# YuxuanZhao/NewsRecommend

Hardware: NVIDIA B200
Metric: queries/s, top-50 IP over 364k x 250 items (flat exact search) (higher is better)
Workload: dtype f32 (fp16 tcgen05 filter with a proven error margin + exact fp32 rescoring)

## Files before the change

newsrecommend_b200/csrc/api.cu:

```cuda
#include <atomic>
#include <cstdarg>
#include <cstdlib>
#include <cstring>
#include <random>
#include <vector>

#include <cuda_fp16.h>

#include "common.cuh"
#include "internal.h"

namespace nrb {

static thread_local char g_err[512] = "";
static std::atomic<long long> g_launches{0};

void set_error(const char* fmt, ...) {
    va_list ap;
    va_start(ap, fmt);
    vsnprintf(g_err, sizeof(g_err), fmt, ap);
    va_end(ap);
}
void count_launch(int n) { g_launches += n; }

// ... 30 lines not shown
    size_t off = 0;
    explicit Carver(void* p) : base((char*)p) {}
    template <typename T>
    T* take(size_t count) {
        T* r = (T*)(base ? base + off : nullptr);
        off += align_up(count * sizeof(T), 256);
        return r;
    }
};

struct FlatPlan {
    int nqt;
    int npairs;
    int full_pairs;
    int tail_pairs;
    int tsplit;
    int chunk_rows;
    int n_units;
    int wgs;
    int S;
    int grid;
    int single;
    int pw;
};

static FlatPlan plan_flat(int64_t nq, int64_t nb, int k, int path) {
    FlatPlan p;
    p.pw = (path == NRB_PATH_TC1 || path == NRB_PATH_TC16) ? tc1_pw(k, nb > 4096) : k;
    const bool simt = path == NRB_PATH_SIMT;
    p.wgs = simt ? 1 : 2;
    p.nqt = (int)((nq + UNIT_ROWS - 1) / UNIT_ROWS);
    if (p.nqt < 1) p.nqt = 1;
    p.npairs = (p.nqt + 1) / 2;
    const int C = simt ? sm_count() : sm_count() / 2;
    const int tile = 256;
    int nbt = (int)((nb + tile - 1) / tile);
    if (nbt < 1) nbt = 1;
    p.full_pairs = (p.npairs / C) * C;
    p.tail_pairs = p.npairs - p.full_pairs;
    int best = 1;
    if (p.tail_pairs > 0) {
        int max_split = nbt < 64 ? nbt : 64;
        static const double ov_tiles = getenv("NRB_FLAT_OV_TILES") ? atof(getenv("NRB_FLAT_OV_TILES")) : 200.0;
        const double ov = ov_tiles / nbt;
        double best_cost = 1e30;
        for (int s = 1; s <= max_split; s++) {
            const double waves = (double)(((int64_t)p.tail_pairs * s + C - 1) / C);
            const double cost = waves * (1.0 / s + ov);
            if (cost < best_cost * 0.97) {
// ... 7 lines not shown
        const int C1 = sm_count();
        static const double ov_tiles1 = getenv("NRB_FLAT_OV_TILES") ? atof(getenv("NRB_FLAT_OV_TILES")) : 200.0;
        const double ov = ov_tiles1 / nbt;
        const int max_split = nbt < 64 ? nbt : 64;
        const double pair_cost = (double)(((int64_t)p.tail_pairs * best + C - 1) / C) * (1.0 / best + ov);
        int best1 = 1;
        double best_cost1 = 1e30;
        for (int s = 1; s <= max_split; s++) {
            const double waves = (double)(((int64_t)p.nqt * s + C1 - 1) / C1);
            const double cost = waves * (1.0 / s + ov);
            if (cost < best_cost1 * 0.97) {
                best_cost1 = cost;
                best1 = s;
            }
        }
        if (best_cost1 < 0.9 * pair_cost || getenv("NRB_FORCE_SINGLE_CTA")) {
            p.single = 1;
            best = best1;
        }
    }
    const int tiles_per = (nbt + best - 1) / best;
    p.chunk_rows = tiles_per * tile;
    p.tsplit = (nbt + tiles_per - 1) / tiles_per;
    p.n_units = p.single ? p.nqt * p.tsplit : 2 * (p.full_pairs + p.tail_pairs * p.tsplit);
    p.S = p.tsplit * p.wgs;
    if (p.single)
        p.grid = p.n_units < sm_count() ? p.n_units : sm_count();
    else
        p.grid = simt ? simt_grid(p.n_units) : tc_grid(p.n_units);
    return p;
}

struct FlatWs {
    Unit* units;
    int* n_units;
    int* src;
    float* part_key;
    int* part_idx;
    int* part_cnt;
    int *flags, *flag_list, *flag_count;
    unsigned* gthr;
    void* scratch;
    size_t scratch_bytes;
    size_t total;
};

static FlatWs carve_flat(void* ws, const FlatPlan& p, int64_t nq, int k, int path) {
    Carver c(ws);
    FlatWs w;
    const bool filt = path == NRB_PATH_TC1 || path == NRB_PATH_TC16;
    const int pw = p.pw;
    w.units = c.take<Unit>(p.n_units);
    w.n_units = c.take<int>(1);
// ... 361 lines not shown
    if (path == NRB_PATH_AUTO)
        path = tc16_eligible(q, b, k) ? NRB_PATH_TC16 : tc1_eligible(q, b, k) ? NRB_PATH_TC1 : NRB_PATH_TC;
    if (path == NRB_PATH_TC1 && !tc1_eligible(q, b, k)) {
        set_error("search_flat: NRB_PATH_TC1 needs raw/hi/norms planes on both sides, max_norm on the item "
                  "side, kp <= 256 and k <= %d", TC1_MAX_PW - TC1_MIN_EXTRA);
        return NRB_ERR_INVALID;
    }
    if (path == NRB_PATH_TC16 && !tc16_eligible(q, b, k)) {
        set_error("search_flat: NRB_PATH_TC16 needs raw/h16/norms planes and h16 scales on both sides, max_norm on "
                  "the item side, kp <= 256 and k <= %d", TC1_MAX_PW - TC1_MIN_EXTRA);
        return NRB_ERR_INVALID;
    }
    const bool filt = path == NRB_PATH_TC1 || path == NRB_PATH_TC16;
    if (!filt) path = resolve_path(path);
    const FlatPlan p = plan_flat(q->n, b->n, k, path);
    const FlatWs w = carve_flat(workspace, p, q->n, k, path);
    if (!workspace || workspace_bytes < w.total) {
        set_error("search_flat: workspace %zu < %zu bytes", workspace_bytes, w.total);
        return NRB_ERR_WORKSPACE;
    }
    int rc;
    if (p.single)
        rc = launch_fill_flat_units_single(w.units, w.n_units, w.src, q->n, b->n, p.nqt, p.tsplit, p.chunk_rows, p.wgs, st);
    else
        rc = launch_fill_flat_units(w.units, w.n_units, w.src, q->n, b->n, p.nqt, p.full_pairs, p.tail_pairs, p.tsplit,
                                    p.chunk_rows, p.wgs, st);
    if (rc) return rc;
    const bool seeded = seed_kth && filt && w.gthr;
    if (seeded) {
        int64_t blocks = (q->n + 255) / 256;
        if (blocks > 148 * 8) blocks = 148 * 8;
        seed_bounds_kernel<<<(unsigned)blocks, 256, 0, st>>>(seed_kth, q->n, metric == NRB_METRIC_L2 ? 1 : 0, w.gthr);
        NRB_LAUNCH_CHECK();
    } else if (w.gthr) {
        NRB_CUDA_CHECK(cudaMemsetAsync(w.gthr, 0, (size_t)q->n * sizeof(unsigned), st));
    }
    if (!filt) {
        {
            ProfScope prof(st);
            if (path == NRB_PATH_SIMT)
                rc = launch_topk_simt_dev(q, b, w.units, w.n_units, p.grid, metric, k, w.part_key, w.part_idx, w.scratch, w.scratch_bytes, st);
            else
                rc = launch_topk_tc_dev(q, b, w.units, w.n_units, p.grid, metric, k, w.part_key, w.part_idx, w.scratch,
                                        w.scratch_bytes, w.gthr, nullptr, 1, st);
        }
        if (rc) return rc;
        return launch_select(w.part_key, w.part_idx, w.src, p.S, q->n, k, metric, nullptr, id_base, D, I, st);
    }
    const int pw = p.pw;
    const float eps_xmax = TC1_EPS * b->max_norm;
    NRB_CUDA_CHECK(cudaMemsetAsync(w.flags, 0, (size_t)q->n * sizeof(int), st));
    {
        ProfScope prof(st);
        rc = launch_topk_tc1_dev(q, b, w.units, w.n_units, p.grid, metric, k, pw, 2.f * eps_xmax, w.part_key,
                                 w.part_idx, w.part_cnt, w.flags, w.scratch, w.scratch_bytes, w.gthr, nullptr, 1,
                                 path == NRB_PATH_TC16, p.single, (!p.single && b->n <= 256) ? 1 : 0, st,
                                 seeded ? 1 : 0);
    }
    if (rc) return rc;
    if ((rc = launch_gather_refine(w.part_key, w.part_idx, w.part_cnt, w.src, p.S, q->n, k, pw, metric, q, b, eps_xmax,
                                   id_base, nullptr, w.flags, D, I, st))) return rc;
    if ((rc = launch_compact_flags(w.flags, q->n, w.flag_list, w.flag_count, st))) return rc;
    if (k == 1 && b->n <= K1_FALLBACK_MAX_ROWS) {
        return launch_exact_k1_fallback(q, b, metric, id_base, w.flag_list, w.flag_count, D, I, st);
    }
    int nflag = 0;
    NRB_CUDA_CHECK(cudaMemcpyAsync(&nflag, w.flag_count, sizeof(int), cudaMemcpyDeviceToHost, st));
    NRB_CUDA_CHECK(cudaStreamSynchronize(st));
    if (nflag == 0) return NRB_OK;
    NRB_REQUIRE(b->hi && b->lo && ((q->hi && q->lo) || q->raw),
                "search_flat: %d queries need the 3xTF32 fallback but the item hi/lo planes are missing", nflag);
    g_fallback_queries += nflag;
    const size_t plane = (size_t)nflag * q->kp * sizeof(float);
    const size_t wsb2 = nrb_search_flat_workspace(nflag, b->n, k, q->kp);
    char* tmp = nullptr;
    const size_t tmp_bytes = 3 * align_up(plane, 256) + align_up((size_t)nflag * 4, 256) +
                             align_up((size_t)nflag * k * 4, 256) + align_up((size_t)nflag * k * 8, 256) + wsb2;
    keep_pool_memory();
    NRB_CUDA_CHECK(cudaMallocAsync((void**)&tmp, tmp_bytes, st));
    Carver c(tmp);
// ... 48 lines not shown
                                      size_t workspace_bytes, int32_t path, const float* seed_kth, void* stream) {
    NRB_REQUIRE(q && b && D && I, "search_flat_seeded: null argument");
    NRB_REQUIRE(metric == NRB_METRIC_INNER_PRODUCT || metric == NRB_METRIC_L2, "search_flat_seeded: bad metric %d", metric);
    NRB_REQUIRE(k >= 1 && k <= NRB_MAX_K, "search_flat_seeded: k=%d out of range [1,%d]", k, NRB_MAX_K);
    NRB_REQUIRE(q->d == b->d && q->kp == b->kp, "search_flat_seeded: dimension mismatch");
    NRB_REQUIRE(q->n >= 0 && b->n >= 0 && b->n < (1LL << 31) - 4096 && q->n < (1LL << 31), "search_flat_seeded: sizes out of range");
    NRB_REQUIRE(path >= NRB_PATH_AUTO && path <= NRB_PATH_TC16, "search_flat_seeded: bad path %d", path);
    if (q->n == 0) return NRB_OK;
    int rc = require_device();
    if (rc) return rc;
    return search_flat_impl(q, b, metric, k, id_base, D, I, workspace, workspace_bytes, path, (cudaStream_t)stream, seed_kth);
}

extern "C" int64_t nrb_fallback_query_count(void) { return (int64_t)g_fallback_queries.load(); }

extern "C" int nrb_plan_flat_describe(int64_t nq, int64_t nb, int32_t k, int32_t path, int32_t* out10) {
    NRB_REQUIRE(out10 && nq >= 1 && nb >= 0 && k >= 1 && k <= NRB_MAX_K, "plan_flat_describe: bad arguments");
    NRB_REQUIRE(path == NRB_PATH_SIMT || path == NRB_PATH_TC || path == NRB_PATH_TC1 || path == NRB_PATH_TC16,
                "plan_flat_describe: path must be a concrete path, not %d", path);
    const FlatPlan p = plan_flat(nq, nb, k, path);
    const int v[10] = {p.nqt, p.npairs, p.full_pairs, p.tail_pairs, p.tsplit, p.chunk_rows, p.n_units, p.S, p.grid, p.single};
    for (int i = 0; i < 10; i++) out10[i] = v[i];
    return NRB_OK;
}

extern "C" size_t nrb_ivf_search_workspace(int64_t nq, int32_t nprobe, int32_t k, int32_t kp,
                                           int32_t nlist, int32_t max_list_len) {
    if (nq <= 0 || nprobe <= 0 || k <= 0) return 256;
    size_t best = 0;
    for (int path : {NRB_PATH_TC, NRB_PATH_SIMT, NRB_PATH_TC16}) {
        if (path == NRB_PATH_TC16 && !tc1_k_ok(k)) continue;
        const IvfPlan p = plan_ivf(nq, nprobe, nlist, max_list_len, path);
        const size_t t = carve_ivf(nullptr, p, nlist, k, kp, path, nq).total;
        best = t > best ? t : best;
    }
    return best + 256;
}

namespace nrb {

static inline int ivf_mode_of(int nph, int i) {
    static const int force = getenv("NRB_IVF_MODE") ? atoi(getenv("NRB_IVF_MODE")) : -1;
    if (force >= 0) return force;
    return (nph > 1 && i == 1) ? 2 : 1;
}

// ... 307 lines not shown
```

newsrecommend_b200/csrc/internal.h:

```cpp
#pragma once
#include <cstdlib>
#include <cuda_runtime.h>
#include <stdint.h>

#include "../../include/nrb200.h"

namespace nrb {

struct Unit {
    int a_row0;
    int a_rows;
    int b_row0;
    int b_rows;
};

constexpr int UNIT_ROWS = 128;

int tc_available();
size_t tc_scratch_bytes(int grid);
int tc_grid(int n_units_upper);
void tc_set_variant(int v);
int launch_topk_tc_dev(const nrb_matrix* a, const nrb_matrix* b, const Unit* units,
                       const int* n_units_dev, int grid, int metric, int k, float* part_key,
                       int* part_idx, void* scratch, size_t scratch_bytes, unsigned* gthr,
                       const int* row_map, int row_div, cudaStream_t st);

constexpr int TC1_EXTRA = 32;
constexpr int TC1_EXTRA_FLAT = 96;
constexpr int TC1_MIN_EXTRA = 16;
constexpr int TC1_MAX_PW = 128;
static inline int tc1_extra() {
    static const int v = getenv("NRB_TC1_EXTRA") ? atoi(getenv("NRB_TC1_EXTRA")) : TC1_EXTRA;
    return v < TC1_MIN_EXTRA ? TC1_MIN_EXTRA : v;
}
static inline int tc1_pw(int k, bool flat = false) {
    const int extra = (flat && !getenv("NRB_TC1_EXTRA")) ? TC1_EXTRA_FLAT : tc1_extra();
    return k + extra <= TC1_MAX_PW ? k + extra : TC1_MAX_PW;
}
static inline int tc1_k_ok(int k) { return k + TC1_MIN_EXTRA <= TC1_MAX_PW; }
constexpr float TC1_EPS = 1.1f / 1024.f;
int tc1_eligible(const nrb_matrix* a, const nrb_matrix* b, int k);
int tc16_eligible(const nrb_matrix* a, const nrb_matrix* b, int k);
int launch_topk_tc1_dev(const nrb_matrix* a, const nrb_matrix* b, const Unit* units,
                        const int* n_units_dev, int grid, int metric, int k, int pw, float margin_scale,
                        float* part_key, int* part_idx, int* part_cnt, int* row_flags, void* scratch,
                        size_t scratch_bytes, unsigned* gthr, const int* row_map, int row_div, int f16,
                        int single, int ivf_mode, cudaStream_t st, int seeded = 0);

size_t simt_scratch_bytes(int grid);
int simt_grid(int n_units_upper);
int launch_topk_simt_dev(const nrb_matrix* a, const nrb_matrix* b, const Unit* units,
                         const int* n_units_dev, int grid, int metric, int k, float* part_key,
                         int* part_idx, void* scratch, size_t scratch_bytes, cudaStream_t st);

int launch_select(const float* part_key, const int* part_idx, const int* src, int S, int64_t nq,
                  int k, int metric, const int64_t* id_map, int64_t id_base, float* D, int64_t* I,
                  cudaStream_t st);
int launch_gather_refine(const float* part_key, const int* part_idx, const int* part_cnt, const int* src, int S,
                         int64_t nq, int k, int pw, int metric, const nrb_matrix* q, const nrb_matrix* b, float eps_xmax,
                         int64_t id_base, const int64_t* id_map, int* flags, float* D, int64_t* I, cudaStream_t st);
int launch_compact_flags(const int* flags, int64_t n, int* list, int* count, cudaStream_t st);
int launch_scatter_results(const float* Df, const int64_t* If, const int* list, int n, int k, float* D,
                           int64_t* I, cudaStream_t st);
int launch_fill_flat_units(Unit* units, int* n_units_out, int* src, int64_t nq, int64_t nb, int nqt,
                           int full_pairs, int tail_pairs, int tsplit, int chunk_rows, int wgs, cudaStream_t st);
int launch_fill_flat_units_single(Unit* units, int* n_units_out, int* src, int64_t nq, int64_t nb, int nqt,
                                  int tsplit, int chunk_rows, int wgs, cudaStream_t st);
size_t counting_sort_ws(int64_t n, int nb);
int launch_counting_sort_i64(const int64_t* key, int64_t n, int nb, int* offsets, int* order,
                             int* pos_of, void* ws, size_t ws_bytes, cudaStream_t st);
int launch_pack_rows(const float* x, int64_t n, int d, int64_t ldx, int kp, float* raw, float* hi, float* lo,
                     float* norms, cudaStream_t st);
int launch_gather_rows(const float* src, int width, const int32_t* idx, int div, int64_t n,
                       float* dst, cudaStream_t st);
int launch_gather_scalar(const float* src, const int32_t* idx, int div, int64_t n, float* dst,
                         cudaStream_t st);

size_t kmeans_update_ws(int64_t n, int k, int kp);
int launch_kmeans_update(const float* x_raw, int64_t n, int d, int kp, const int64_t* assign, int k, float* centroids,
                         float* hassign, void* workspace, const float* cent_in, int metric, double* obj_out,
                         cudaStream_t st, double* sums_out = nullptr);
int launch_km_split(int d, int k, int64_t n, float* hassign, float* centroids, double* stats, cudaStream_t st);

constexpr int K1_FALLBACK_MAX_ROWS = 65536;
int launch_exact_k1_fallback(const nrb_matrix* q, const nrb_matrix* b, int metric, int64_t id_base, const int* list,
                             const int* count, float* D, int64_t* I, cudaStream_t st);

int sm_count();
// ... 3 lines not shown
```

newsrecommend_b200/csrc/kernels_misc.cu:

```cuda
#include <cfloat>

#include <cuda_fp16.h>

#include "common.cuh"
#include "internal.h"

namespace nrb {

__global__ void pack_rows_kernel(const float* __restrict__ x, int64_t n, int d, int64_t ldx,
                                 int kp, float* __restrict__ raw, float* __restrict__ hi,
                                 float* __restrict__ lo, float* __restrict__ norms) {
    const int lane = threadIdx.x & 31;
    const int64_t warp0 = (int64_t)blockIdx.x * (blockDim.x >> 5) + (threadIdx.x >> 5);
    const int64_t nwarps = (int64_t)gridDim.x * (blockDim.x >> 5);
    for (int64_t row = warp0; row < n; row += nwarps) {
        const float* xr = x + row * ldx;
        float acc = 0.f;
        for (int c = lane; c < kp; c += 32) {
            float v = (c < d) ? xr[c] : 0.f;
            acc = fmaf(v, v, acc);
            const int64_t o = row * kp + c;
            if (raw) raw[o] = v;
            if (hi || lo) {
                uint32_t hb, lb;
// ... 881 lines not shown
            u.b_row0 = c * chunk_rows;
            const int64_t br = nb - (int64_t)c * chunk_rows;
            u.b_rows = (int)(br < chunk_rows ? (br > 0 ? br : 0) : chunk_rows);
        }
        units[tid] = u;
    }
    const int S = tsplit * wgs;
    const int64_t total = nq * S;
    for (int64_t e = tid; e < total; e += (int64_t)gridDim.x * blockDim.x) {
        const int64_t q = e / S;
        const int sl = (int)(e - q * S);
        const int c = sl / wgs, g = sl - c * wgs;
        const int t = (int)(q / UNIT_ROWS), pair = t >> 1, r = t & 1;
        int64_t u = -1;
        if (pair < full_pairs) {
            if (c == 0) u = 2 * (int64_t)pair + r;
        } else {
            u = 2 * ((int64_t)full_pairs + (int64_t)c * tail_pairs + (pair - full_pairs)) + r;
        }
        src[e] = u < 0 ? -1 : (int)((u * wgs + g) * UNIT_ROWS + q % UNIT_ROWS);
    }
}

__global__ void fill_flat_units_single_kernel(Unit* __restrict__ units, int* __restrict__ n_units_out,
                                              int* __restrict__ src, int64_t nq, int64_t nb, int nqt, int tsplit,
                                              int chunk_rows, int wgs) {
    const int64_t tid = (int64_t)blockIdx.x * blockDim.x + threadIdx.x;
    const int64_t nunits = (int64_t)nqt * tsplit;
    if (tid == 0) *n_units_out = (int)nunits;
    if (tid < nunits) {
        const int c = (int)(tid / nqt), t = (int)(tid - (int64_t)c * nqt);
        Unit u;
        const int64_t ar = nq - (int64_t)t * UNIT_ROWS;
        u.a_rows = (int)(ar < UNIT_ROWS ? ar : UNIT_ROWS);
        u.a_row0 = t * UNIT_ROWS;
        u.b_row0 = c * chunk_rows;
        const int64_t br = nb - (int64_t)c * chunk_rows;
        u.b_rows = (int)(br < chunk_rows ? (br > 0 ? br : 0) : chunk_rows);
        units[tid] = u;
    }
    const int S = tsplit * wgs;
    const int64_t total = nq * S;
    for (int64_t e = tid; e < total; e += (int64_t)gridDim.x * blockDim.x) {
        const int64_t q = e / S;
        const int sl = (int)(e - q * S);
        const int c = sl / wgs, g = sl - c * wgs;
// ... 50 lines not shown
    return NRB_OK;
}

int launch_scatter_results(const float* Df, const int64_t* If, const int* list, int n, int k, float* D,
                           int64_t* I, cudaStream_t st) {
    if (n == 0) return NRB_OK;
    int64_t blocks = ((int64_t)n * k + 255) / 256;
    if (blocks > 4096) blocks = 4096;
    scatter_results_kernel<<<(unsigned)blocks, 256, 0, st>>>(Df, If, list, n, k, D, I);
    NRB_LAUNCH_CHECK();
    return NRB_OK;
}

int launch_fill_flat_units(Unit* units, int* n_units_out, int* src, int64_t nq, int64_t nb, int nqt,
                           int full_pairs, int tail_pairs, int tsplit, int chunk_rows, int wgs, cudaStream_t st) {
    const int64_t total = nq * tsplit * wgs;
    const int64_t nunits = 2 * ((int64_t)full_pairs + (int64_t)tail_pairs * tsplit);
    int64_t blocks = (total + 255) / 256;
    if (blocks > 4096) blocks = 4096;
    if (blocks < (nunits + 255) / 256) blocks = (nunits + 255) / 256;
    if (blocks < 1) blocks = 1;
    fill_flat_units_kernel<<<(unsigned)blocks, 256, 0, st>>>(units, n_units_out, src, nq, nb, nqt, full_pairs,
                                                             tail_pairs, tsplit, chunk_rows, wgs);
    NRB_LAUNCH_CHECK();
    return NRB_OK;
}

int launch_fill_flat_units_single(Unit* units, int* n_units_out, int* src, int64_t nq, int64_t nb, int nqt,
                                  int tsplit, int chunk_rows, int wgs, cudaStream_t st) {
    const int64_t total = nq * tsplit * wgs;
    const int64_t nunits = (int64_t)nqt * tsplit;
    int64_t blocks = (total + 255) / 256;
    if (blocks > 4096) blocks = 4096;
    if (blocks < (nunits + 255) / 256) blocks = (nunits + 255) / 256;
    if (blocks < 1) blocks = 1;
    fill_flat_units_single_kernel<<<(unsigned)blocks, 256, 0, st>>>(units, n_units_out, src, nq, nb, nqt, tsplit,
                                                                    chunk_rows, wgs);
    NRB_LAUNCH_CHECK();
    return NRB_OK;
}

size_t counting_sort_ws(int64_t n, int nb);
int launch_counting_sort_i64(const int64_t* key, int64_t n, int nb, int* offsets, int* order,
                             int* pos_of, void* ws, size_t ws_bytes, cudaStream_t st) {
    const int nchunks = (int)((n + CS_CHUNK - 1) / CS_CHUNK);
    const size_t need = counting_sort_ws(n, nb);
// ... 364 lines not shown
```

newsrecommend_b200/csrc/topk_tc.cu:

```cuda
#include <cuda.h>

#include <cstdlib>

#include "common.cuh"
#include "internal.h"
#include "ptx.cuh"

namespace nrb {

namespace {

constexpr int BM = 128;
constexpr int BN = 256;
constexpr int KC = 32;
constexpr int A_BYTES = BM * KC * 4;
constexpr int BH_BYTES = (BN / 2) * KC * 4;
constexpr int B_BYTES = BN * KC * 4;
constexpr int NUM_THREADS = 384;
constexpr int EPI_WARP0 = 4;
constexpr int EPI_WGS = 2;
constexpr int HALF_N = BN / EPI_WGS;
constexpr int TMEM_COLS = 512;

constexpr int V1_STAGES = 2;
// ... 13 lines not shown
};

template <int STAGES>
struct TcShared {
    uint64_t full[STAGES];
    uint64_t empty[STAGES];
    uint64_t tfull[2];
    uint64_t tempty[2];
    uint32_t tmem_base;
    uint32_t pad;
    float nrm[EPI_WGS][2][HALF_N];
    XchgShared xchg;
};

constexpr size_t V1_SMEM = (size_t)V1_STAGES * V1_STAGE_BYTES + sizeof(TcShared<V1_STAGES>) + 1024;
constexpr size_t V2_SMEM = (size_t)V2_STAGES * V2_STAGE_BYTES + sizeof(TcShared<V2_STAGES>) + 1024;

#ifdef NRB_TRACE
constexpr int NRB_TRACE_TILES = 4096;
__device__ long long g_trace[9][NRB_TRACE_TILES][4];
__device__ long long g_trace_prune[9][64][4];
__device__ int g_trace_prune_n[9];
__device__ int g_trace_enable = 1;
#define NRB_TRP(who, ev)                                                                                   \
    do {                                                                                                   \
        if (blockIdx.x == 0 && (threadIdx.x & 31) == 0 && g_trace_enable && g_trace_prune_n[who] < 64)      \
            g_trace_prune[who][g_trace_prune_n[who]][ev] = clock64();                                      \
    } while (0)
#define NRB_TRP_NEXT(who)                                                                           \
    do {                                                                                            \
        if (blockIdx.x == 0 && (threadIdx.x & 31) == 0 && g_trace_enable) g_trace_prune_n[who]++; \
    } while (0)
#define NRB_TR(who, tile, ev)                                                                                      \
    do {                                                                                                           \
        if (blockIdx.x == 0 && (threadIdx.x & 31) == 0 && g_trace_enable && (tile) < (uint32_t)NRB_TRACE_TILES)      \
            g_trace[who][tile][ev] = clock64();                                                                    \
    } while (0)
#else
#define NRB_TR(who, tile, ev) \
    do {                      \
    } while (0)
#define NRB_TRP(who, ev) \
    do {                 \
    } while (0)
#define NRB_TRP_NEXT(who) \
    do {                  \
// ... 467 lines not shown
    }
}

struct EpiArgs {
    const Unit* units;
    int n_units, k, pw;
    float margin_scale;
    const float *a_norms, *b_norms;
    int64_t a_total, b_total;
    float* part_key;
    int* part_idx;
    int* part_cnt;
    int* row_flags;
    uint2* cand_buf;
    unsigned* gthr;
    const int* row_map;
    int row_div;
    const float* a_row_scale;
    float b_scale;
    int hot;
    int one_shot_ok;
    int seeded;
    int first_shot_ok;
};
#ifndef NRB_HOT_MIN_TILES
#define NRB_HOT_MIN_TILES (1 << 30)
#endif
constexpr int HOT_MIN_TILES = NRB_HOT_MIN_TILES;

template <bool L2, bool PAIR, bool NEED_QN, bool IVFX = false>
__device__ __forceinline__ void epilogue_run(const EpiArgs& A, uint64_t* tfull, uint64_t* tempty,
                                             float (*nrm)[2][HALF_N], XchgShared* xs, uint32_t tmem_base, int warp,
                                             int lane, uint32_t rank) {
    const int wg = (warp - EPI_WARP0) >> 2;
    const int quad = warp & 3;
    const int row = quad * 32 + lane;
    const int etid = ((warp - EPI_WARP0) & 3) * 32 + lane;
    const int64_t crow0 = ((int64_t)blockIdx.x * EPI_WGS + wg) * BM + quad * 32;
    uint2* cb = A.cand_buf + crow0 * CAND_CAP;
    uint2* myb = cb + (int64_t)lane * CAND_CAP;
    uint32_t tempty_remote0 = 0, tempty_remote1 = 0;
    if (PAIR) {
        tempty_remote0 = ptx::mapa_u32(&tempty[0], 0);
        tempty_remote1 = ptx::mapa_u32(&tempty[1], 0);
    }
    const int first = PAIR ? (int)(blockIdx.x >> 1) : (int)blockIdx.x;
    const int stride = PAIR ? (int)(gridDim.x >> 1) : (int)gridDim.x;
    const int count = PAIR ? (A.n_units + 1) >> 1 : A.n_units;
    const uint32_t taddr_wg = tmem_base + ((uint32_t)(quad * 32) << 16) + (uint32_t)(wg * HALF_N);
    uint32_t gt = 0;
    for (int i = first; i < count; i += stride) {
        const int u = PAIR ? 2 * i + (int)rank : i;
        const Unit un = A.units[u];
        const int ntiles = (PAIR || un.a_rows > 0) ? (un.b_rows + BN - 1) / BN : 0;
        const int64_t ar = (int64_t)un.a_row0 + row;
        const bool live = row < un.a_rows && ar < A.a_total;
        EpiRow st;
        st.cnt = 0;
        st.base = 0;
        st.thr = live ? NEG_INF : __builtin_huge_valf();
        st.cthr = st.thr;
        st.sc = (A.a_row_scale && live) ? A.a_row_scale[ar] * A.b_scale : 1.f;
        st.inv = 1.f / st.sc;
        st.qn = ((L2 || NEED_QN) && live) ? A.a_norms[ar] : 0.f;
        st.margin = NEED_QN ? A.margin_scale * sqrtf(st.qn) * (L2 ? 2.f : 1.f) : 0.f;
        st.flag = 0;
        st.gslot = nullptr;
        if (A.gthr && live) st.gslot = A.gthr + (A.row_map ? A.row_map[ar] / A.row_div : (int)ar);
        const bool hot = IVFX && A.hot;
        const bool one_shot = IVFX && NEED_QN && !hot && ntiles == 1 && A.one_shot_ok;
        bool first_shot = false;
        if (NEED_QN && !hot && ntiles > 1 && A.first_shot_ok && !A.seeded) {
            unsigned g0 = 0u;
            if (st.gslot) g0 = *(volatile unsigned*)st.gslot;
            if (wg == 0)
                xs->nthr[row] = g0 != 0u ? 1.f : 0.f;
            else
                xs->lb[row] = g0 != 0u ? 1u : 0u;
            ptx::named_bar_sync(3 + quad, 64);
            const bool warm = xs->nthr[row] != 0.f || xs->lb[row] != 0u;
            first_shot = !__any_sync(0xffffffffu, warm);
        }
        for (int t = 0; t < ntiles; t++, gt++) {
            const int acc = (int)(gt & 1);
            const uint32_t acc_phase = (gt >> 1) & 1;
            const int col_base = t * BN + wg * HALF_N;
            const int valid = un.b_rows - col_base;
            unsigned g_raw = 0;
            if (st.gslot) g_raw = *(volatile unsigned*)st.gslot;
            float* nrm_t = nrm[wg][acc];
            epi_stage_norms<L2>(nrm_t, A.b_norms, un, col_base, valid, A.b_total, etid, wg);
            NRB_TR(warp - EPI_WARP0 + 1, gt, 0);
            ptx::mbar_wait(&tfull[acc], acc_phase);
            ptx::tcgen05_fence_after();
            NRB_TR(warp - EPI_WARP0 + 1, gt, 1);
            if (st.gslot) {
                st.thr = fmaxf(st.thr, from_ordered_u32(g_raw) - st.margin);
                st.cthr = L2 ? st.thr + st.qn : st.thr * st.sc;
            }
            const uint32_t taddr0 = taddr_wg + (uint32_t)(acc * BN);
            auto release = [&]() {
                ptx::tcgen05_fence_before();
                __syncwarp();
                if (lane == 0) {
                    if (PAIR)
                        ptx::mbar_arrive_cluster_relaxed(acc ? tempty_remote1 : tempty_remote0);
                    else
                        ptx::mbar_arrive(&tempty[acc]);
                }
            };
            if ((IVFX && one_shot) || (first_shot && t == 0)) {
                const OneShotOut o = single_tile_call<L2, PAIR>(taddr0, valid, un.b_row0 + col_base, nrm_t, st.sc, st.inv, st.qn,
                                                              st.margin, myb, A.k, xs, wg, row, quad,
                                                              acc ? tempty_remote1 : tempty_remote0, &tempty[acc]);
                st.cnt = live ? o.cnt : 0;
// ... 32 lines not shown
                xs->fresh[wg][row] = st.cnt - st.base;
                xs->thr[wg][row] = st.thr;
                if (wg == 0) xs->margin[row] = st.margin;
                NRB_TRP(warp - EPI_WARP0 + 1, 0);
                ptx::named_bar_sync(3 + quad, 64);
                NRB_TRP(warp - EPI_WARP0 + 1, 1);
                union_tighten_rows(xs, A.cand_buf + (int64_t)blockIdx.x * EPI_WGS * BM * CAND_CAP, quad, wg, A.k, A.pw,
                                   (A.row_map || A.seeded) ? max(4, A.k >> 2) : 0);
                NRB_TRP(warp - EPI_WARP0 + 1, 2);
                ptx::named_bar_sync(3 + quad, 64);
                NRB_TRP(warp - EPI_WARP0 + 1, 3);
                NRB_TRP_NEXT(warp - EPI_WARP0 + 1);
                if (xs->done[row]) {
                    st.cnt = xs->cnt[wg][row];
                    st.base = st.cnt;
                    st.thr = xs->nthr[row];
                    st.cthr = L2 ? st.thr + st.qn : st.thr * st.sc;
                    const uint32_t lbu = xs->lb[row];
                    if (wg == 0 && st.gslot && lbu != 0u) atomicMax(st.gslot, lbu);
                    if (NEED_QN && xs->ovf[row] && live) epi_abandon_row(st);
                }
            }
        }
        if (IVFX && NEED_QN && (hot || one_shot)) {
            const unsigned need = __ballot_sync(0xffffffffu, st.cnt > A.pw);
            if (need) epi_prune_rows<L2>(need, st, cb, A.k, A.pw, lane);
            if (st.cnt > A.pw) {
                st.flag = 1;
                st.cnt = A.pw;
            }
            epi_unit_end_unsorted(live ? st.cnt : 0, cb, ((int64_t)u * EPI_WGS + wg) * UNIT_ROWS + quad * 32, A.pw,
                                  A.part_key, A.part_idx, A.part_cnt, lane);
        } else if (NEED_QN) {
            xs->cnt[wg][row] = st.cnt;
            xs->fresh[wg][row] = st.cnt - st.base;
            xs->thr[wg][row] = st.thr;
            if (wg == 0) xs->margin[row] = st.margin;
            ptx::named_bar_sync(3 + quad, 64);
            union_tighten_rows(xs, A.cand_buf + (int64_t)blockIdx.x * EPI_WGS * BM * CAND_CAP, quad, wg, A.k, A.pw, -1);
            ptx::named_bar_sync(3 + quad, 64);
            if (xs->done[row]) {
                st.cnt = xs->cnt[wg][row];
                const uint32_t lbu = xs->lb[row];
                if (wg == 0 && st.gslot && lbu != 0u) atomicMax(st.gslot, lbu);
                if (xs->ovf[row] && live) epi_abandon_row(st);
            }
            if (st.cnt > A.pw) {
                st.flag = 1;
                st.cnt = A.pw;
            }
            epi_unit_end_unsorted(live ? st.cnt : 0, cb, ((int64_t)u * EPI_WGS + wg) * UNIT_ROWS + quad * 32, A.pw,
                                  A.part_key, A.part_idx, A.part_cnt, lane);
        } else {
            epi_unit_end(st, cb, ((int64_t)u * EPI_WGS + wg) * UNIT_ROWS + quad * 32, A.k, A.pw, A.part_key, A.part_idx, lane);
        }
        if (NEED_QN && st.flag && live) A.row_flags[A.row_map ? A.row_map[ar] / A.row_div : (int)ar] = 1;
    }
}

template <bool L2>
__global__ void __launch_bounds__(NUM_THREADS, 1)
topk_tc_kernel(const __grid_constant__ CUtensorMap map_ah, const __grid_constant__ CUtensorMap map_al,
               const __grid_constant__ CUtensorMap map_bh, const __grid_constant__ CUtensorMap map_bl,
               const Unit* __restrict__ units, const int* __restrict__ n_units_p, int nkc, int k,
               const float* __restrict__ a_norms, const float* __restrict__ b_norms,
               int64_t a_total, int64_t b_total, float* __restrict__ part_key,
               int* __restrict__ part_idx, float* __restrict__ cand_key_buf,
               int* __restrict__ cand_idx_buf, unsigned* __restrict__ gthr, const int* __restrict__ row_map,
               int row_div) {
    constexpr int STAGES = V1_STAGES, STAGE_BYTES = V1_STAGE_BYTES;
    extern __shared__ uint8_t smem_raw[];
    uint8_t* smem = reinterpret_cast<uint8_t*>((reinterpret_cast<uintptr_t>(smem_raw) + 1023) & ~(uintptr_t)1023);
    TcShared<STAGES>* sh = reinterpret_cast<TcShared<STAGES>*>(smem + (size_t)STAGES * STAGE_BYTES);

    const int warp = threadIdx.x >> 5, lane = threadIdx.x & 31;
    const int n_units = *n_units_p;

    if (threadIdx.x == 0) {
        for (int s = 0; s < STAGES; s++) {
// ... 450 lines not shown
                    if (ptx::elect_one()) {
                        if (PAIR)
                            ptx::umma_commit_cg2_mc(&sh->tfull[acc], 3);
                        else
                            ptx::umma_commit(&sh->tfull[acc]);
                    }
                    __syncwarp();
                    NRB_TR(0, mma_gt, 1);
                    acc ^= 1;
                    if (acc == 0) acc_phase ^= 1;
                }
                if (ptx::elect_one()) {
                    if (PAIR)
                        ptx::umma_commit_cg2_mc(&sh->aempty[ab], 3);
                    else
                        ptx::umma_commit(&sh->aempty[ab]);
                }
                __syncwarp();
            }
        }
    } else if (warp >= EPI_WARP0) {
        ptx::setmaxnreg_inc<232>();
        EpiArgs ea{units, *n_units_p, k, pw, margin_scale, a_norms, b_norms, a_total, b_total, part_key, part_idx,
                   part_cnt, row_flags, reinterpret_cast<uint2*>(cand_key_buf), gthr, row_map, row_div, a_row_scale, b_scale, hot & 1, (hot & 2) ? 0 : 1, (hot & 4) ? 1 : 0, (hot & 8) ? 0 : 1};
        epilogue_run<L2, PAIR, true, A2>(ea, sh->tfull, sh->tempty, sh->nrm, &sh->xchg, tmem_base, warp, lane, rank);
    }

    ptx::tcgen05_fence_before();
    if (PAIR) {
        __syncwarp();
        ptx::cluster_sync_all();
    } else {
        __syncthreads();
    }
    if (warp == 1) {
        ptx::tcgen05_fence_after();
        if (PAIR)
            ptx::tmem_dealloc_cg2(tmem_base, TMEM_COLS);
        else
            ptx::tmem_dealloc(tmem_base, TMEM_COLS);
    }
}

#define NRB_TC3_PARAMS                                                                                              \
    const __grid_constant__ CUtensorMap map_ah, const __grid_constant__ CUtensorMap map_bh,                         \
        const Unit *__restrict__ units, const int *__restrict__ n_units_p, int nkc, int k, int pw, float margin_scale, \
        const float *__restrict__ a_norms, const float *__restrict__ b_norms, int64_t a_total, int64_t b_total,    \
// ... 154 lines not shown
            NRB_TC_LAUNCH(topk_tc2_kernel<true>, V2_SMEM);
        else
            NRB_TC_LAUNCH(topk_tc2_kernel<false>, V2_SMEM);
    }
#undef NRB_TC_LAUNCH
    NRB_LAUNCH_CHECK();
    return NRB_OK;
}

int tc1_eligible(const nrb_matrix* a, const nrb_matrix* b, int k) {
    return a->hi && b->hi && a->raw && b->raw && a->norms && b->norms && b->max_norm > 0.f &&
           a->kp == b->kp && a->kp <= V3_MAX_NKC * KC && tc1_k_ok(k);
}

int tc16_eligible(const nrb_matrix* a, const nrb_matrix* b, int k) {
    return a->h16 && a->h16_row_scale && b->h16 && b->h16_scale > 0.f && a->raw && b->raw && a->norms &&
           b->norms && b->max_norm > 0.f && a->kp == b->kp && a->kp <= V3_MAX_NKC * KC && tc1_k_ok(k);
}

int launch_topk_tc1_dev(const nrb_matrix* a, const nrb_matrix* b, const Unit* units,
                        const int* n_units_dev, int grid, int metric, int k, int pw, float margin_scale,
                        float* part_key, int* part_idx, int* part_cnt, int* row_flags, void* scratch,
                        size_t scratch_bytes, unsigned* gthr, const int* row_map, int row_div, int f16,
                        int single, int ivf_mode, cudaStream_t st, int seeded) {
    static const int no_one_shot = (getenv("NRB_NO_ONE_SHOT") ? 2 : 0) | (getenv("NRB_NO_FIRST_SHOT") ? 8 : 0);
    const int hot = (ivf_mode == 2 ? 1 : 0) | no_one_shot | (seeded ? 4 : 0);
    NRB_REQUIRE(part_cnt, "tc1: part_cnt required (the filter kernels write unsorted partial rows)");
    NRB_REQUIRE(!single || f16, "tc1: the single-CTA form exists for the fp16 planes only");
    if (f16)
        NRB_REQUIRE(a->h16 && a->h16_row_scale && b->h16 && b->h16_scale > 0.f, "tc16: scaled fp16 planes required");
    else
        NRB_REQUIRE(a->hi && b->hi, "tc1: hi planes required");
    NRB_REQUIRE(a->norms && b->norms && a->kp == b->kp && a->kp <= V3_MAX_NKC * KC && tc1_k_ok(k) && row_div >= 1,
                "tc1: norms on both sides, kp <= 256 and k <= %d required", TC1_MAX_PW - TC1_MIN_EXTRA);
    NRB_REQUIRE(a->kp % KC == 0 && pw >= k && pw <= CAND_CAP - HALF_N, "tc1: bad kp / pw");
    NRB_REQUIRE(grid >= 1 && (single || grid % 2 == 0), "tc1: grid must be positive (and even for CTA pairs)");
    if (scratch_bytes < tc_scratch_bytes(grid)) {
        set_error("tc1: scratch too small");
        return NRB_ERR_WORKSPACE;
    }
#ifdef NRB_TRACE
    {
        const char* e = getenv("NRB_TRACE_IVF_MODE");
        const int en = (!e || atoi(e) == ivf_mode) ? 1 : 0;
        NRB_CUDA_CHECK(cudaMemcpyToSymbolAsync(g_trace_enable, &en, sizeof(int), 0, cudaMemcpyHostToDevice, st));
    }
#endif
    CUtensorMap mah, mbh;
    int rc;
// ... 60 lines not shown
    return NRB_OK;
}

}

#ifdef NRB_TRACE
extern "C" int nrb_debug_trace_read(void* host_buf, size_t bytes) {
    const size_t have = sizeof(long long) * 9 * nrb::NRB_TRACE_TILES * 4;
    if (bytes < have) return -1;
    if (cudaDeviceSynchronize() != cudaSuccess) return -2;
    return cudaMemcpyFromSymbol(host_buf, nrb::g_trace, have) == cudaSuccess ? 0 : -2;
}
extern "C" int nrb_debug_trace_prune_read(void* host_buf, size_t bytes, int reset) {
    const size_t have = sizeof(long long) * 9 * 64 * 4;
    if (bytes < have) return -1;
    if (cudaDeviceSynchronize() != cudaSuccess) return -2;
    if (cudaMemcpyFromSymbol(host_buf, nrb::g_trace_prune, have) != cudaSuccess) return -2;
    if (reset) {
        int z[9] = {0};
        cudaMemcpyToSymbol(nrb::g_trace_prune_n, z, sizeof(z));
    }
    return 0;
}
#endif
```

Measured before the change: 5.809 million.

## Schedule tail query pairs with uneven hot item chunks and cache flat plans

Adds a planner that, for the partial final wave of CTA-pair units, splits the item range into uneven chunks. A long cold head chunk goes to the leftover slot and shorter later chunks go to CTAs that already hold a warmed top-k threshold, balancing estimated per-CTA makespan with a simple cost model. The epilogue gains a hot mode for non-IVF units: when every row already has a threshold it runs the in-place prune path. Flat plans are also cached under a mutex to avoid recomputing the layout search per call. This adds planner complexity and cost-model constants that may mispredict real makespan, plus trace instrumentation.

```diff
diff --git a/newsrecommend_b200/csrc/api.cu b/newsrecommend_b200/csrc/api.cu
--- a/newsrecommend_b200/csrc/api.cu
+++ b/newsrecommend_b200/csrc/api.cu
@@ -1,4 +1,6 @@
+#include <algorithm>
 #include <atomic>
+#include <mutex>
 #include <cstdarg>
 #include <cstdlib>
 #include <cstring>
@@ -76,9 +78,94 @@
     int grid;
     int single;
     int pw;
+    int hot;
+    FlatTail tail;
 };
 
-static FlatPlan plan_flat(int64_t nq, int64_t nb, int k, int path) {
+static double flat_equal_makespan(int C, int F, int T, int s, int nbt, int tiles_per, double ov_cold) {
+    std::vector<double> load(C, 0.0);
+    for (int i = 0; i < F + T * s; i++) {
+        const int c = i < F ? -1 : (i - F) / T;
+        const int len = c < 0 ? nbt : std::min(tiles_per, nbt - c * tiles_per);
+        load[i % C] += len + ov_cold;
+    }
+    return *std::max_element(load.begin(), load.end());
+}
+
+static double flat_hot_layout(int C, int F, int T, int s, int nbt, int64_t nb, int H, double ov_cold, double hot_rate,
+                              double ov_hot, FlatTail* out) {
+    if (T < 1 || T >= C || F < C || F % C || s < 2 || T * s > FLAT_TAIL_MAX) return -1;
+    const int f = F / C, npu = F + T * s;
+    const int lmax = (int)((nb - 1) / (256 * (int64_t)(s - 1)));
+    if (H < 1 || H > lmax || nbt - H < s - 1) return -1;
+    std::vector<int> n(C), h(C);
+    int Q = 0;
+    for (int j = 0; j < C; j++) {
+        n[j] = (npu - j + C - 1) / C;
+        if (n[j] > f) Q = j + 1;
+    }
+    const int hs0 = Q - T;
+    if (hs0 < 0) return -1;
+    auto head = [&](int j) { return j >= hs0 && j < hs0 + T; };
+    double sum_fixed = 0.0;
+    int nhot_slots = 0;
+    for (int j = 0; j < C; j++) {
+        h[j] = n[j] - f - (head(j) ? 1 : 0);
+        if (h[j] > 0) {
+            sum_fixed += (head(j) ? H + ov_cold : 0.0) + h[j] * ov_hot;
+            nhot_slots++;
+        }
+    }
+    if (nhot_slots == 0) return -1;
+    const double M = (hot_rate * T * (nbt - H) + sum_fixed) / nhot_slots;
+    struct Pos {
+        double target;
+        int slot, k;
+    };
+    std::vector<Pos> pos;
+    for (int j = 0; j < C; j++)
+        for (int k = 0; k < h[j]; k++)
+            pos.push_back({std::max(1.0, (M - (head(j) ? H + ov_cold : 0.0) - h[j] * ov_hot) / (h[j] * hot_rate)), j, k});
+    std::stable_sort(pos.begin(), pos.end(), [](const Pos& a, const Pos& b) { return a.target > b.target; });
+    std::vector<std::vector<int>> mine(T);
+    std::vector<double> sum(T, 0.0);
+    for (int i = 0; i < (int)pos.size(); i++) {
+        int best = -1;
+        for (int j = 0; j < T; j++)
+            if ((int)mine[j].size() < s - 1 && (best < 0 || sum[j] < sum[best])) best = j;
+        mine[best].push_back(i);
+        sum[best] += pos[i].target;
+    }
+    std::vector<double> load(C);
+    for (int j = 0; j < C; j++) load[j] = f * (nbt + ov_cold) + (head(j) ? H + ov_cold : 0.0);
+    out->C = C;
+    out->F = F;
+    out->T = T;
+    out->s = s;
+    out->nbt = nbt;
+    out->hs0 = hs0;
+    out->hot_first = 0;
+    for (int j = 0; j < T; j++) {
+        out->unit[j * s] = hs0 + j;
+        out->tile0[j * s] = 0;
+        int start = H;
+        double cum = 0.0;
+        for (int c = 1; c < s; c++) {
+            const Pos& ps = pos[mine[j][c - 1]];
+            cum += ps.target;
+            const int end = c == s - 1 ? nbt : H + (int)llround((nbt - H) * cum / sum[j]);
+            const int len = end - start;
+            if (len < 1 || len > lmax) return -1;
+            out->unit[j * s + c] = ps.slot + (f + (head(ps.slot) ? 1 : 0) + ps.k) * C;
+            out->tile0[j * s + c] = start;
+            load[ps.slot] += hot_rate * len + ov_hot;
+            start = end;
+        }
+    }
+    return *std::max_element(load.begin(), load.end());
+}
+
+static FlatPlan plan_flat_uncached(int64_t nq, int64_t nb, int k, int path) {
     FlatPlan p;
     p.pw = (path == NRB_PATH_TC1 || path == NRB_PATH_TC16) ? tc1_pw(k, nb > 4096) : k;
     const bool simt = path == NRB_PATH_SIMT;
@@ -132,6 +219,45 @@
     const int tiles_per = (nbt + best - 1) / best;
     p.chunk_rows = tiles_per * tile;
     p.tsplit = (nbt + tiles_per - 1) / tiles_per;
+    p.hot = 0;
+    const bool filt = path == NRB_PATH_TC1 || path == NRB_PATH_TC16;
+    if (filt && !p.single && p.full_pairs > 0 && p.tail_pairs > 0 && !getenv("NRB_FLAT_EQUAL_CHUNKS")) {
+        static const double ov_cold = getenv("NRB_FLAT_OV_TILES") ? atof(getenv("NRB_FLAT_OV_TILES")) : 200.0;
+        static const double hot_rate = getenv("NRB_FLAT_HOT_TILE_COST") ? atof(getenv("NRB_FLAT_HOT_TILE_COST")) : 0.8;
+        static const double ov_hot = getenv("NRB_FLAT_HOT_OV_TILES") ? atof(getenv("NRB_FLAT_HOT_OV_TILES")) : 24.0;
+        double best_ms = flat_equal_makespan(C, p.full_pairs, p.tail_pairs, p.tsplit, nbt, tiles_per, ov_cold);
+        FlatTail cand;
+        for (int s = 2; s <= 4; s++) {
+            const int lmax = (int)((nb - 1) / (256 * (int64_t)(s - 1)));
+            for (int i = 0; i <= 8; i++) {
+                const int H = (int)(((int64_t)lmax * (16 - i) + 15) / 16);
+                const double ms = flat_hot_layout(C, p.full_pairs, p.tail_pairs, s, nbt, nb, H, ov_cold, hot_rate, ov_hot, &cand);
+                if (ms > 0 && ms < best_ms * 0.99) {
+                    best_ms = ms;
+                    p.hot = 1;
+                    p.tail = cand;
+                }
+            }
+        }
+        if (p.hot) {
+            const FlatTail& t = p.tail;
+            int longest = 0;
+            for (int i = 0; i < t.T * t.s; i++) {
+                const int end = (i % t.s == t.s - 1) ? t.nbt : t.tile0[i + 1];
+                longest = std::max(longest, end - t.tile0[i]);
+            }
+            p.tsplit = t.s;
+            p.chunk_rows = longest * tile;
+            if (getenv("NRB_FLAT_HOT_FIRST")) {
+                p.tail.hot_first = 1;
+                const int npu = t.F + t.T * t.s;
+                for (int i = 0; i < t.T * t.s; i++) {
+                    const int j = t.unit[i] % t.C, pos = t.unit[i] / t.C, nj = (npu - j + t.C - 1) / t.C;
+                    p.tail.unit[i] = j + (nj - 1 - pos) * t.C;
+                }
+            }
+        }
+    }
     p.n_units = p.single ? p.nqt * p.tsplit : 2 * (p.full_pairs + p.tail_pairs * p.tsplit);
     p.S = p.tsplit * p.wgs;
     if (p.single)
@@ -139,6 +265,28 @@
     else
         p.grid = simt ? simt_grid(p.n_units) : tc_grid(p.n_units);
     return p;
+}
+
+static FlatPlan plan_flat(int64_t nq, int64_t nb, int k, int path) {
+    constexpr int N = 8;
+    struct Entry {
+        int64_t key[5];
+        FlatPlan plan;
+    };
+    static std::mutex mu;
+    static Entry cache[N];
+    static int used = 0, next = 0;
+    const int64_t key[5] = {nq, nb, k, path,
+                            (getenv("NRB_FLAT_HOT_FIRST") ? 1 : 0) | (getenv("NRB_FLAT_EQUAL_CHUNKS") ? 2 : 0)};
+    std::lock_guard<std::mutex> lock(mu);
+    for (int i = 0; i < used; i++)
+        if (!memcmp(cache[i].key, key, sizeof(key))) return cache[i].plan;
+    Entry& e = cache[next];
+    memcpy(e.key, key, sizeof(key));
+    e.plan = plan_flat_uncached(nq, nb, k, path);
+    next = (next + 1) % N;
+    used = used < N ? used + 1 : N;
+    return e.plan;
 }
 
 struct FlatWs {
@@ -546,6 +694,8 @@
     int rc;
     if (p.single)
         rc = launch_fill_flat_units_single(w.units, w.n_units, w.src, q->n, b->n, p.nqt, p.tsplit, p.chunk_rows, p.wgs, st);
+    else if (p.hot)
+        rc = launch_fill_flat_units_hot(w.units, w.n_units, w.src, q->n, b->n, p.nqt, p.tail, p.wgs, st);
     else
         rc = launch_fill_flat_units(w.units, w.n_units, w.src, q->n, b->n, p.nqt, p.full_pairs, p.tail_pairs, p.tsplit,
                                     p.chunk_rows, p.wgs, st);
@@ -579,7 +729,7 @@
         rc = launch_topk_tc1_dev(q, b, w.units, w.n_units, p.grid, metric, k, pw, 2.f * eps_xmax, w.part_key,
                                  w.part_idx, w.part_cnt, w.flags, w.scratch, w.scratch_bytes, w.gthr, nullptr, 1,
                                  path == NRB_PATH_TC16, p.single, (!p.single && b->n <= 256) ? 1 : 0, st,
-                                 seeded ? 1 : 0);
+                                 seeded ? 1 : 0, p.hot);
     }
     if (rc) return rc;
     if ((rc = launch_gather_refine(w.part_key, w.part_idx, w.part_cnt, w.src, p.S, q->n, k, pw, metric, q, b, eps_xmax,
@@ -674,6 +824,22 @@
     const int v[10] = {p.nqt, p.npairs, p.full_pairs, p.tail_pairs, p.tsplit, p.chunk_rows, p.n_units, p.S, p.grid, p.single};
     for (int i = 0; i < 10; i++) out10[i] = v[i];
     return NRB_OK;
+}
+
+extern "C" int nrb_debug_plan_flat_layout(int64_t nq, int64_t nb, int32_t k, int32_t path, int32_t* out, int32_t cap) {
+    NRB_REQUIRE(out && nq >= 1 && nb >= 1 && k >= 1 && k <= NRB_MAX_K, "plan_flat_layout: bad arguments");
+    const FlatPlan p = plan_flat(nq, nb, k, path);
+    if (!p.hot) return 0;
+    const FlatTail& t = p.tail;
+    const int n = t.F + t.T * t.s;
+    if (cap < n) return -1;
+    for (int L = 0; L < n; L++) {
+        int t0, t1;
+        const int pu = flat_tail_piece(t, L, &t0, &t1);
+        const int v[5] = {pu, L < t.F ? L : t.F + (L - t.F) / t.s, L < t.F ? 0 : (L - t.F) % t.s, t0, t1};
+        for (int i = 0; i < 5; i++) out[5 * L + i] = v[i];
+    }
+    return n;
 }
 
 extern "C" size_t nrb_ivf_search_workspace(int64_t nq, int32_t nprobe, int32_t k, int32_t kp,
diff --git a/newsrecommend_b200/csrc/internal.h b/newsrecommend_b200/csrc/internal.h
--- a/newsrecommend_b200/csrc/internal.h
+++ b/newsrecommend_b200/csrc/internal.h
@@ -45,7 +45,7 @@
                         const int* n_units_dev, int grid, int metric, int k, int pw, float margin_scale,
                         float* part_key, int* part_idx, int* part_cnt, int* row_flags, void* scratch,
                         size_t scratch_bytes, unsigned* gthr, const int* row_map, int row_div, int f16,
-                        int single, int ivf_mode, cudaStream_t st, int seeded = 0);
+                        int single, int ivf_mode, cudaStream_t st, int seeded = 0, int hot_units = 0);
 
 size_t simt_scratch_bytes(int grid);
 int simt_grid(int n_units_upper);
@@ -64,6 +64,31 @@
                            int64_t* I, cudaStream_t st);
 int launch_fill_flat_units(Unit* units, int* n_units_out, int* src, int64_t nq, int64_t nb, int nqt,
                            int full_pairs, int tail_pairs, int tsplit, int chunk_rows, int wgs, cudaStream_t st);
+constexpr int FLAT_TAIL_MAX = 296;
+struct FlatTail {
+    int C, F, T, s;
+    int nbt;
+    int hs0;
+    int hot_first;
+    int unit[FLAT_TAIL_MAX];
+    int tile0[FLAT_TAIL_MAX];
+};
+__host__ __device__ inline int flat_tail_piece(const FlatTail& t, int L, int* t0, int* t1) {
+    if (L < t.F) {
+        const int j = L % t.C;
+        int p = L / t.C + ((j >= t.hs0 && j < t.hs0 + t.T) ? 1 : 0);
+        if (t.hot_first) p = (t.F + t.T * t.s - j + t.C - 1) / t.C - 1 - p;
+        *t0 = 0;
+        *t1 = t.nbt;
+        return j + p * t.C;
+    }
+    const int P = L - t.F;
+    *t0 = t.tile0[P];
+    *t1 = (P % t.s == t.s - 1) ? t.nbt : t.tile0[P + 1];
+    return t.unit[P];
+}
+int launch_fill_flat_units_hot(Unit* units, int* n_units_out, int* src, int64_t nq, int64_t nb, int nqt,
+                               const FlatTail& tail, int wgs, cudaStream_t st);
 int launch_fill_flat_units_single(Unit* units, int* n_units_out, int* src, int64_t nq, int64_t nb, int nqt,
                                   int tsplit, int chunk_rows, int wgs, cudaStream_t st);
 size_t counting_sort_ws(int64_t n, int nb);
diff --git a/newsrecommend_b200/csrc/kernels_misc.cu b/newsrecommend_b200/csrc/kernels_misc.cu
--- a/newsrecommend_b200/csrc/kernels_misc.cu
+++ b/newsrecommend_b200/csrc/kernels_misc.cu
@@ -927,6 +927,45 @@
     }
 }
 
+__global__ void fill_flat_units_hot_kernel(Unit* __restrict__ units, int* __restrict__ n_units_out,
+                                           int* __restrict__ src, int64_t nq, int64_t nb, int nqt, const FlatTail tail,
+                                           int wgs) {
+    const int64_t tid = (int64_t)blockIdx.x * blockDim.x + threadIdx.x;
+    const int64_t nunits = 2 * ((int64_t)tail.F + (int64_t)tail.T * tail.s);
+    if (tid == 0) *n_units_out = (int)nunits;
+    if (tid < nunits) {
+        const int L = (int)(tid >> 1), r = (int)(tid & 1);
+        const int pair = L < tail.F ? L : tail.F + (L - tail.F) / tail.s;
+        int t0, t1;
+        const int pu = flat_tail_piece(tail, L, &t0, &t1);
+        const int t = 2 * pair + r;
+        Unit u;
+        const int64_t ar = nq - (int64_t)t * UNIT_ROWS;
+        u.a_rows = t < nqt ? (int)(ar < UNIT_ROWS ? ar : UNIT_ROWS) : 0;
+        u.a_row0 = t < nqt ? t * UNIT_ROWS : 0;
+        u.b_row0 = t0 * 256;
+        const int64_t br = (t1 * 256 < nb ? (int64_t)t1 * 256 : nb) - (int64_t)t0 * 256;
+        u.b_rows = (int)br;
+        units[2 * pu + r] = u;
+    }
+    const int S = tail.s * wgs;
+    const int64_t total = nq * S;
+    for (int64_t e = tid; e < total; e += (int64_t)gridDim.x * blockDim.x) {
+        const int64_t q = e / S;
+        const int sl = (int)(e - q * S);
+        const int c = sl / wgs, g = sl - c * wgs;
+        const int t = (int)(q / UNIT_ROWS), pair = t >> 1, r = t & 1;
+        int64_t u = -1;
+        int t0, t1;
+        if (pair < tail.F) {
+            if (c == 0) u = 2 * (int64_t)flat_tail_piece(tail, pair, &t0, &t1) + r;
+        } else {
+            u = 2 * (int64_t)flat_tail_piece(tail, tail.F + (pair - tail.F) * tail.s + c, &t0, &t1) + r;
+        }
+        src[e] = u < 0 ? -1 : (int)((u * wgs + g) * UNIT_ROWS + q % UNIT_ROWS);
+    }
+}
+
 __global__ void fill_flat_units_single_kernel(Unit* __restrict__ units, int* __restrict__ n_units_out,
                                               int* __restrict__ src, int64_t nq, int64_t nb, int nqt, int tsplit,
                                               int chunk_rows, int wgs) {
@@ -1023,6 +1062,19 @@
     if (blocks < 1) blocks = 1;
     fill_flat_units_kernel<<<(unsigned)blocks, 256, 0, st>>>(units, n_units_out, src, nq, nb, nqt, full_pairs,
                                                              tail_pairs, tsplit, chunk_rows, wgs);
+    NRB_LAUNCH_CHECK();
+    return NRB_OK;
+}
+
+int launch_fill_flat_units_hot(Unit* units, int* n_units_out, int* src, int64_t nq, int64_t nb, int nqt,
+                               const FlatTail& tail, int wgs, cudaStream_t st) {
+    const int64_t total = nq * tail.s * wgs;
+    const int64_t nunits = 2 * ((int64_t)tail.F + (int64_t)tail.T * tail.s);
+    int64_t blocks = (total + 255) / 256;
+    if (blocks > 4096) blocks = 4096;
+    if (blocks < (nunits + 255) / 256) blocks = (nunits + 255) / 256;
+    if (blocks < 1) blocks = 1;
+    fill_flat_units_hot_kernel<<<(unsigned)blocks, 256, 0, st>>>(units, n_units_out, src, nq, nb, nqt, tail, wgs);
     NRB_LAUNCH_CHECK();
     return NRB_OK;
 }
diff --git a/newsrecommend_b200/csrc/topk_tc.cu b/newsrecommend_b200/csrc/topk_tc.cu
--- a/newsrecommend_b200/csrc/topk_tc.cu
+++ b/newsrecommend_b200/csrc/topk_tc.cu
@@ -59,6 +59,13 @@
 __device__ long long g_trace_prune[9][64][4];
 __device__ int g_trace_prune_n[9];
 __device__ int g_trace_enable = 1;
+constexpr int NRB_TRACE_UNITS = 8192;
+__device__ long long g_trace_units[NRB_TRACE_UNITS][6];
+__device__ __forceinline__ long long trace_globaltimer() {
+    long long t;
+    asm volatile("mov.u64 %0, %%globaltimer;" : "=l"(t));
+    return t;
+}
 #define NRB_TRP(who, ev)                                                                                   \
     do {                                                                                                   \
         if (blockIdx.x == 0 && (threadIdx.x & 31) == 0 && g_trace_enable && g_trace_prune_n[who] < 64)      \
@@ -572,6 +579,7 @@
     int one_shot_ok;
     int seeded;
     int first_shot_ok;
+    int hot_ok;
 };
 #ifndef NRB_HOT_MIN_TILES
 #define NRB_HOT_MIN_TILES (1 << 30)
@@ -617,10 +625,10 @@
         st.flag = 0;
         st.gslot = nullptr;
         if (A.gthr && live) st.gslot = A.gthr + (A.row_map ? A.row_map[ar] / A.row_div : (int)ar);
-        const bool hot = IVFX && A.hot;
+        bool hot = IVFX && A.hot;
         const bool one_shot = IVFX && NEED_QN && !hot && ntiles == 1 && A.one_shot_ok;
         bool first_shot = false;
-        if (NEED_QN && !hot && ntiles > 1 && A.first_shot_ok && !A.seeded) {
+        if (NEED_QN && !hot && ntiles > 1 && (A.first_shot_ok || (!IVFX && A.hot_ok)) && !A.seeded) {
             unsigned g0 = 0u;
             if (st.gslot) g0 = *(volatile unsigned*)st.gslot;
             if (wg == 0)
@@ -629,7 +637,11 @@
                 xs->lb[row] = g0 != 0u ? 1u : 0u;
             ptx::named_bar_sync(3 + quad, 64);
             const bool warm = xs->nthr[row] != 0.f || xs->lb[row] != 0u;
-            first_shot = !__any_sync(0xffffffffu, warm);
+            first_shot = A.first_shot_ok && !__any_sync(0xffffffffu, warm);
+            if (!IVFX && A.hot_ok) {
+                hot = __all_sync(0xffffffffu, warm || !live);
+                ptx::named_bar_sync(3 + quad, 64);
+            }
         }
         for (int t = 0; t < ntiles; t++, gt++) {
             const int acc = (int)(gt & 1);
@@ -641,6 +653,15 @@
             float* nrm_t = nrm[wg][acc];
             epi_stage_norms<L2>(nrm_t, A.b_norms, un, col_base, valid, A.b_total, etid, wg);
             NRB_TR(warp - EPI_WARP0 + 1, gt, 0);
+#ifdef NRB_TRACE
+            if (t == 0 && warp == EPI_WARP0 && lane == 0 && rank == 0 && g_trace_enable && i < NRB_TRACE_UNITS) {
+                g_trace_units[i][0] = first;
+                g_trace_units[i][1] = i;
+                g_trace_units[i][2] = trace_globaltimer();
+                g_trace_units[i][4] = ntiles;
+                g_trace_units[i][5] = hot ? 1 : 0;
+            }
+#endif
             ptx::mbar_wait(&tfull[acc], acc_phase);
             ptx::tcgen05_fence_after();
             NRB_TR(warp - EPI_WARP0 + 1, gt, 1);
@@ -719,7 +740,7 @@
                 }
             }
         }
-        if (IVFX && NEED_QN && (hot || one_shot)) {
+        if (NEED_QN && (hot || one_shot)) {
             const unsigned need = __ballot_sync(0xffffffffu, st.cnt > A.pw);
             if (need) epi_prune_rows<L2>(need, st, cb, A.k, A.pw, lane);
             if (st.cnt > A.pw) {
@@ -752,6 +773,10 @@
             epi_unit_end(st, cb, ((int64_t)u * EPI_WGS + wg) * UNIT_ROWS + quad * 32, A.k, A.pw, A.part_key, A.part_idx, lane);
         }
         if (NEED_QN && st.flag && live) A.row_flags[A.row_map ? A.row_map[ar] / A.row_div : (int)ar] = 1;
+#ifdef NRB_TRACE
+        if (ntiles > 0 && warp == EPI_WARP0 && lane == 0 && rank == 0 && g_trace_enable && i < NRB_TRACE_UNITS)
+            g_trace_units[i][3] = trace_globaltimer();
+#endif
     }
 }
 
@@ -1248,7 +1273,7 @@
     } else if (warp >= EPI_WARP0) {
         ptx::setmaxnreg_inc<232>();
         EpiArgs ea{units, *n_units_p, k, pw, margin_scale, a_norms, b_norms, a_total, b_total, part_key, part_idx,
-                   part_cnt, row_flags, reinterpret_cast<uint2*>(cand_key_buf), gthr, row_map, row_div, a_row_scale, b_scale, hot & 1, (hot & 2) ? 0 : 1, (hot & 4) ? 1 : 0, (hot & 8) ? 0 : 1};
+                   part_cnt, row_flags, reinterpret_cast<uint2*>(cand_key_buf), gthr, row_map, row_div, a_row_scale, b_scale, hot & 1, (hot & 2) ? 0 : 1, (hot & 4) ? 1 : 0, (hot & 8) ? 0 : 1, (hot & 16) ? 1 : 0};
         epilogue_run<L2, PAIR, true, A2>(ea, sh->tfull, sh->tempty, sh->nrm, &sh->xchg, tmem_base, warp, lane, rank);
     }
 
@@ -1449,9 +1474,9 @@
                         const int* n_units_dev, int grid, int metric, int k, int pw, float margin_scale,
                         float* part_key, int* part_idx, int* part_cnt, int* row_flags, void* scratch,
                         size_t scratch_bytes, unsigned* gthr, const int* row_map, int row_div, int f16,
-                        int single, int ivf_mode, cudaStream_t st, int seeded) {
+                        int single, int ivf_mode, cudaStream_t st, int seeded, int hot_units) {
     static const int no_one_shot = (getenv("NRB_NO_ONE_SHOT") ? 2 : 0) | (getenv("NRB_NO_FIRST_SHOT") ? 8 : 0);
-    const int hot = (ivf_mode == 2 ? 1 : 0) | no_one_shot | (seeded ? 4 : 0);
+    const int hot = (ivf_mode == 2 ? 1 : 0) | no_one_shot | (seeded ? 4 : 0) | (hot_units && ivf_mode == 0 ? 16 : 0);
     NRB_REQUIRE(part_cnt, "tc1: part_cnt required (the filter kernels write unsorted partial rows)");
     NRB_REQUIRE(!single || f16, "tc1: the single-CTA form exists for the fp16 planes only");
     if (f16)
@@ -1558,4 +1583,14 @@
     }
     return 0;
 }
+extern "C" int nrb_debug_units_read(void* host_buf, size_t bytes, int reset) {
+    const size_t have = sizeof(long long) * nrb::NRB_TRACE_UNITS * 6;
+    if (bytes < have) return -1;
+    if (cudaDeviceSynchronize() != cudaSuccess) return -2;
+    if (cudaMemcpyFromSymbol(host_buf, nrb::g_trace_units, have) != cudaSuccess) return -2;
+    void* dev = nullptr;
+    if (reset && (cudaGetSymbolAddress(&dev, nrb::g_trace_units) != cudaSuccess || cudaMemset(dev, 0, have) != cudaSuccess))
+        return -2;
+    return 0;
+}
 #endif
```

Measured after the change: 5.978 million, median of 6. +2.9%, better.
